# zpelgrims/pota

Measured on AMD Instinct MI355X. Metric: bidir redistribution Msamples/s at 4K, double-gauss 50mm, higher is better.
Workload: dtype f64

## Files before the change

### include/lentil_hip.h

```cpp
#ifndef LENTIL_HIP_H
#define LENTIL_HIP_H

#include <stddef.h>
#include <stdint.h>

#ifdef __cplusplus
extern "C" {
#endif

#define LENTIL_ABI_VERSION 1

#define LENTIL_OK 0
#define LENTIL_ERR_INVALID (-1)
#define LENTIL_ERR_HIP (-2)
#define LENTIL_ERR_UNSUPPORTED (-3)
#define LENTIL_ERR_NOMEM (-4)

#define LENTIL_THINLENS 0
#define LENTIL_POLYNOMIAL_OPTICS 1
#define LENTIL_UNIT_MM 0
#define LENTIL_UNIT_CM 1
#define LENTIL_UNIT_DM 2
#define LENTIL_UNIT_M 3
#define LENTIL_FILTER_GAUSSIAN 0
// ... 331 lines not shown
  uint64_t capacity;
  lentil_draw *out;
  double lambda;
  uint64_t *n_draws;
  uint64_t *attempts;
} lentil_draw_list;
int lentil_hip_list_draws(lentil_hip_ctx *ctx, const lentil_draw_list *list);
int lentil_hip_list_draws_path(lentil_hip_ctx *ctx, int *path);
int lentil_hip_draw_channels(const lentil_params *p, uint32_t *n_channels, double lambda[3], float rgb_weight[3][3]);

int lentil_hip_test_y0_intersection(lentil_hip_ctx *ctx, uint64_t n, const double *sensor_shift, double lambda,
                                    double *distance, double *sensor, double *out);
int lentil_hip_test_lt_sample_aperture(lentil_hip_ctx *ctx, uint64_t n, const double *scene,
                                       const double *ap, double lambda, double *sensor,
                                       double *out, double *transmittance);
int lentil_hip_test_trace_bw_po(lentil_hip_ctx *ctx, uint64_t n, const double *target,
                                const int32_t *px, const int32_t *py, const int32_t *attempt,
                                double *sensor_xy, int32_t *ok);
int lentil_hip_test_aperture_sample(lentil_hip_ctx *ctx, uint64_t n, const uint32_t *a,
                                    const uint32_t *b, double *xy);
int lentil_hip_test_xor128_jump(const uint32_t in[4], uint64_t k, uint32_t out[4]);
int lentil_hip_debug_scan_bands(const lentil_params *params, float out[8]);
int lentil_hip_debug_scan_lean_counts(uint32_t out[3]);
enum {
  LENTIL_SCAN_DMA2 = 1,
  LENTIL_SCAN_DMA = 2,
  LENTIL_SCAN_DMA_MULTI = 3,
  LENTIL_SCAN_UNIFORM = 4,
  LENTIL_SCAN_UNIFORM_MULTI = 5,
  LENTIL_SCAN_RUNS = 6,
// ... 9 lines not shown
```

### pota_amd/capi.py

```python
import ctypes as C
import os

import numpy as np

from . import _abi

_PKG = os.path.dirname(os.path.abspath(__file__))
LIB_PATH = os.environ.get("LENTIL_HIP_LIB") or os.path.join(_PKG, "liblentil_hip.so")

EXPORTS = [
    "lentil_hip_abi_version", "lentil_hip_create", "lentil_hip_destroy", "lentil_hip_last_error", "lentil_hip_last_redo_note",
    "lentil_hip_set_params", "lentil_hip_set_lens", "lentil_hip_set_bokeh", "lentil_hip_alloc_frame", "lentil_hip_set_camera_motion", "lentil_hip_set_camera_shutter",
    "lentil_hip_upload_visits", "lentil_hip_bind_visits", "lentil_hip_clear_frame",
    "lentil_hip_redistribute", "lentil_hip_resolve", "lentil_hip_sync", "lentil_hip_download_aov",
    "lentil_hip_download_accum", "lentil_hip_download_records", "lentil_hip_accum_buffer", "lentil_hip_stream",
    "lentil_hip_set_closest_exchange", "lentil_hip_zkey_buffer", "lentil_hip_closest_gather",
    "lentil_hip_touched_rows", "lentil_hip_merge_rows", "lentil_hip_resolve_rows",
    "lentil_hip_pack_rows", "lentil_hip_merge_packed_rows", "lentil_hip_compact_rows", "lentil_hip_merge_sparse",
    "lentil_hip_get_counters", "lentil_hip_last_timing", "lentil_hip_last_launches", "lentil_hip_set_draw_log",
    "lentil_hip_batch_model_stats", "lentil_hip_process_stats", "lentil_hip_process_stall_notes", "lentil_hip_set_async", "lentil_hip_pass_totals", "lentil_hip_set_occlusion_probe", "lentil_hip_probe_stats",
    "lentil_hip_set_occlusion_probe_device", "lentil_hip_probe_device_stats", "lentil_hip_test_sphere_occluder_device", "lentil_hip_debug_batch_estimate", "lentil_hip_box_probe",
    "lentil_hip_lens_jit_status", "lentil_hip_lens_jit_wait", "lentil_hip_debug_lens_jit_source", "lentil_hip_debug_lens_jit_compile",
    "lentil_hip_download_draw_log", "lentil_hip_test_lt_sample_aperture",
    "lentil_hip_test_trace_bw_po", "lentil_hip_test_aperture_sample", "lentil_hip_debug_scan_bands", "lentil_hip_debug_scan_lean_counts", "lentil_hip_debug_last_scan",
    "lentil_hip_lens_is_compiled", "lentil_hip_set_lens_mode",
    "lentil_hip_focus_search", "lentil_hip_test_y0_intersection", "lentil_hip_camera_rays", "lentil_hip_camera_rays_path",
    "lentil_hip_trace_points", "lentil_hip_trace_points_path",
    "lentil_hip_plan_visits", "lentil_hip_list_draws", "lentil_hip_list_draws_path", "lentil_hip_draw_channels",
    "lentil_hip_set_xor128_state", "lentil_hip_get_xor128_state", "lentil_hip_tl_chroma_stats", "lentil_hip_test_xor128_jump",
    "lentil_hip_host_alloc", "lentil_hip_host_free", "lentil_hip_visits_begin", "lentil_hip_visits_append",
    "lentil_hip_visits_wait", "lentil_hip_visits_end",
    "lentil_hip_comm_unique_id", "lentil_hip_comm_init", "lentil_hip_comm_destroy", "lentil_hip_allreduce",
    "lentil_hip_exchange_bands", "lentil_hip_exchange_stats", "lentil_hip_exchange_counts", "lentil_hip_degenerate_stats", "lentil_hip_streams_concurrent",
    "lentil_hip_alloc_crypto", "lentil_hip_upload_crypto", "lentil_hip_bind_crypto", "lentil_hip_download_crypto",
    "lentil_hip_download_crypto_table", "lentil_hip_visits_begin_crypto", "lentil_hip_visits_append_crypto",
]

SCAN_DMA2, SCAN_DMA, SCAN_DMA_MULTI, SCAN_UNIFORM, SCAN_UNIFORM_MULTI, SCAN_RUNS, SCAN_RAGGED = range(1, 8)
# ... 113 lines not shown
        "lentil_hip_lens_jit_wait": (i, [vp, C.c_double]),
        "lentil_hip_debug_lens_jit_compile": (i, [vp, i, C.c_char_p, C.c_uint64, C.POINTER(C.c_uint64), C.c_char_p, C.c_uint64,
                                                  C.POINTER(C.c_double), C.POINTER(C.c_uint64)]),
        "lentil_hip_debug_lens_jit_source": (i, [vp, C.c_char_p, C.c_uint64, C.POINTER(C.c_uint64)]),
        "lentil_hip_debug_batch_estimate": (i, [vp, C.c_uint64, vp, C.c_uint32, vp]),
        "lentil_hip_alloc_crypto": (i, [vp, u32, u32]),
        "lentil_hip_upload_crypto": (i, [vp, C.POINTER(_abi.CryptoVisits)]),
        "lentil_hip_bind_crypto": (i, [vp, C.POINTER(_abi.CryptoVisits)]),
        "lentil_hip_download_crypto": (i, [vp, u32, u32, vp, vp]),
        "lentil_hip_visits_begin_crypto": (i, [vp, u32]),
        "lentil_hip_visits_append_crypto": (i, [vp, C.POINTER(_abi.Visits), C.POINTER(_abi.CryptoVisits), C.POINTER(u64)]),
        "lentil_hip_download_crypto_table": (i, [vp, u32, C.POINTER(u32), vp, vp, vp]),
        "lentil_hip_set_draw_log": (i, [vp, u64]),
        "lentil_hip_download_draw_log": (i, [vp, vp, u64, C.POINTER(u64)]),
        "lentil_hip_test_lt_sample_aperture": (i, [vp, u64, vp, vp, C.c_double, vp, vp, vp]),
        "lentil_hip_test_trace_bw_po": (i, [vp, u64, vp, vp, vp, vp, vp, vp]),
        "lentil_hip_test_aperture_sample": (i, [vp, u64, vp, vp, vp]),
        "lentil_hip_lens_is_compiled": (i, [vp]),
        "lentil_hip_set_lens_mode": (i, [vp, i]),
        "lentil_hip_focus_search": (i, [vp, C.c_double, C.c_double, C.POINTER(C.c_double)]),
        "lentil_hip_camera_rays": (i, [vp, C.POINTER(_abi.CameraRayBatch)]),
        "lentil_hip_camera_rays_path": (i, [vp, C.POINTER(C.c_int)]),
        "lentil_hip_trace_points": (i, [vp, C.POINTER(_abi.PointBatch)]),
        "lentil_hip_trace_points_path": (i, [vp, C.POINTER(C.c_int)]),
        "lentil_hip_plan_visits": (i, [vp, u64, u64, vp, C.c_uint32, C.POINTER(u64)]),
        "lentil_hip_list_draws": (i, [vp, C.POINTER(_abi.DrawList)]),
        "lentil_hip_list_draws_path": (i, [vp, C.POINTER(C.c_int)]),
        "lentil_hip_draw_channels": (i, [C.POINTER(_abi.Params), C.POINTER(u32), C.POINTER(C.c_double), C.POINTER(C.c_float)]),
        "lentil_hip_set_xor128_state": (i, [vp, C.POINTER(C.c_uint32)]),
        "lentil_hip_get_xor128_state": (i, [vp, C.POINTER(C.c_uint32)]),
# ... 627 lines not shown
        self._chk(self.lib.lentil_hip_download_draw_log(self.h, None, 0, C.byref(n)))
        rec = np.empty((n.value, 3), np.uint32)
        if n.value:
            self._chk(self.lib.lentil_hip_download_draw_log(self.h, rec.ctypes.data, n.value, C.byref(n)))
        return rec

    def test_lt_sample_aperture(self, scene, ap, lam):
        scene = np.ascontiguousarray(scene, np.float64)
        ap = np.ascontiguousarray(ap, np.float64)
        n = scene.shape[0]
        sensor = np.empty((n, 5)); out = np.empty((n, 5)); T = np.empty((n,))
        self._chk(self.lib.lentil_hip_test_lt_sample_aperture(
            self.h, n, scene.ctypes.data, ap.ctypes.data, lam, sensor.ctypes.data, out.ctypes.data, T.ctypes.data))
        return sensor, out, T

    def test_trace_bw_po(self, target, px, py, attempt):
        target = np.ascontiguousarray(target, np.float64)
        px = np.ascontiguousarray(px, np.int32); py = np.ascontiguousarray(py, np.int32)
        attempt = np.ascontiguousarray(attempt, np.int32)
        n = target.shape[0]
        xy = np.empty((n, 2)); ok = np.empty((n,), np.int32)
        self._chk(self.lib.lentil_hip_test_trace_bw_po(
            self.h, n, target.ctypes.data, px.ctypes.data, py.ctypes.data, attempt.ctypes.data,
            xy.ctypes.data, ok.ctypes.data))
        return xy, ok

    def test_aperture_sample(self, a, b):
        a = np.ascontiguousarray(a, np.uint32); b = np.ascontiguousarray(b, np.uint32)
        xy = np.empty((a.shape[0], 2))
        self._chk(self.lib.lentil_hip_test_aperture_sample(self.h, a.shape[0], a.ctypes.data, b.ctypes.data,
# ... 3 lines not shown
```

### pota_amd/csrc/lentil_device.h

```cpp
#pragma once
#include <hip/hip_runtime.h>
#include <stdint.h>

#include "../../include/lentil_hip.h"

#define LD_DEV __device__ __forceinline__

namespace lentil {

constexpr float kAiPi = 3.14159265358979323846f;
constexpr float kAiPiOver2 = 1.57079632679489661923f;
constexpr float kAiEpsilon = 1.0e-4f;
constexpr float kAiInfinite = 1.0e30f;
constexpr double kPi = 3.14159265358979323846;

enum PolyId {
  P_OUT_X = 0, P_OUT_Y, P_OUT_DX, P_OUT_DY, P_OUT_T,
  P_AP_X, P_AP_Y, P_AP_DX, P_AP_DY,
  P_DAP_00, P_DAP_01, P_DAP_10, P_DAP_11,
  P_DOUT_00, P_DOUT_01, P_DOUT_10, P_DOUT_11,
  P_DAPPOS_00, P_DAPPOS_01, P_DAPPOS_10, P_DAPPOS_11,
  P_COUNT
};

// ... 160 lines not shown
  const double n2 = sqrt(fmax(0.0, R * R - ipx * ipx - ipy * ipy)) / fabs(R);
  const double t2 = sqrt(fmax(0.0, 1.0 - idx * idx - idy * idy));
  double ex0 = n2, ex1 = 0.0, ex2 = -n0;
  normalise3(ex0, ex1, ex2);
  const double ey0 = n1 * ex2 - n2 * ex1;
  const double ey1 = n2 * ex0 - n0 * ex2;
  const double ey2 = n0 * ex1 - n1 * ex0;
  dir[0] = idx * ex0 + idy * ey0 + t2 * n0;
  dir[1] = idx * ex1 + idy * ey1 + t2 * n1;
  dir[2] = idx * ex2 + idy * ey2 + t2 * n2;
  pos[0] = ipx;
  pos[1] = ipy;
  pos[2] = n2 * R + center;
}

LD_DEV void csToSphere(const double pos[3], double vx, double vy, double vz, double &odx, double &ody,
                       double center, double R) {
  const double n0 = pos[0] / R, n1 = pos[1] / R, n2 = fabs((pos[2] - center) / R);
  normalise3(vx, vy, vz);
  double ex0 = n2, ex1 = 0.0, ex2 = -n0;
  normalise3(ex0, ex1, ex2);
  const double ey0 = n1 * ex2 - n2 * ex1;
  const double ey1 = n2 * ex0 - n0 * ex2;
  const double ey2 = n0 * ex1 - n1 * ex0;
  odx = vx * ex0 + vy * ex1 + vz * ex2;
  ody = vx * ey0 + vy * ey1 + vz * ey2;
}

LD_DEV void cylinderToCs(double ipx, double ipy, double idx, double idy, double pos[3], double dir[3],
                         double center, double R, bool cyl_y) {
  double n0 = 0.0, n1 = 0.0, n2;
  if (cyl_y) { n0 = ipx / R; n2 = sqrt(fmax(0.0, R * R - ipx * ipx)) / fabs(R); }
  else { n1 = ipy / R; n2 = sqrt(fmax(0.0, R * R - ipy * ipy)) / fabs(R); }
  const double t2 = sqrt(fmax(0.0, 1.0 - idx * idx - idy * idy));
  double ex0 = n2, ex1 = 0.0, ex2 = -n0;
  normalise3(ex0, ex1, ex2);
  double ey0 = n1 * ex2 - n2 * ex1;
  double ey1 = n2 * ex0 - n0 * ex2;
  double ey2 = n0 * ex1 - n1 * ex0;
  normalise3(ey0, ey1, ey2);
  dir[0] = idx * ex0 + idy * ey0 + t2 * n0;
  dir[1] = idx * ex1 + idy * ey1 + t2 * n1;
  dir[2] = idx * ex2 + idy * ey2 + t2 * n2;
  pos[0] = ipx;
  pos[1] = ipy;
  pos[2] = n2 * R + center;
}

LD_DEV void csToCylinder(const double pos[3], double vx, double vy, double vz, double &odx, double &ody,
                         double center, double R, bool cyl_y) {
  double n0 = 0.0, n1 = 0.0;
  if (cyl_y) n0 = pos[0] / R; else n1 = pos[1] / R;
  const double n2 = fabs((pos[2] - center) / R);
  normalise3(vx, vy, vz);
  const double ex0 = n2, ex1 = 0.0, ex2 = -n0;
  double ey0 = n1 * ex2 - n2 * ex1;
  double ey1 = n2 * ex0 - n0 * ex2;
  double ey2 = n0 * ex1 - n1 * ex0;
  normalise3(ey0, ey1, ey2);
  odx = vx * ex0 + vy * ex1 + vz * ex2;
  ody = vx * ey0 + vy * ey1 + vz * ey2;
}

LD_DEV double ipow_u(double x, uint32_t e) {
  uint32_t odd = 0, n = 0;
  while (e > 2) { odd = (odd << 1) | (e & 1u); ++n; e >>= 1; }
  double p = (e == 2) ? x * x : x;
  for (uint32_t i = 0; i < n; ++i) {
    p = (odd & 1u) ? (x * p) * p : p * p;
    odd >>= 1;
  }
  return p;
}

struct LdsLens {
  const DevTerm *terms;
// ... 52 lines not shown
  int k, error;
};

LD_DEV void newton_init(NewtonState &s) {
  s.x = 0; s.y = 0; s.dx = 0; s.dy = 0;
  s.sqr_err = 1e30; s.sqr_ap_err = 1e30;
  s.out[0] = s.out[1] = s.out[2] = s.out[3] = 0.0;
  s.k = 0; s.error = 0;
}

LD_DEV bool newton_continue(const NewtonState &s) {
  const double eps = 1e-8;
  return s.k < 100 && (s.sqr_err > eps || s.sqr_ap_err > eps) && s.error == 0;
}

template <class Lens>
LD_DEV void newton_iter(const Lens &L, const double scene[3], double ap_x, double ap_y, NewtonState &s) {
  const DevLens &k = L.consts();
  const double R = k.outer_pupil_curvature_radius;
  const double prev_sqr_err = s.sqr_err, prev_sqr_ap_err = s.sqr_ap_err;
  const double begin[4] = {s.x, s.y, s.dx, s.dy};
  double pred_ap[2], Jap[4], Jout[4];
  L.eval_bw(begin, pred_ap, Jap, s.out, Jout);
  const double d0 = ap_x - pred_ap[0], d1 = ap_y - pred_ap[1];
  s.sqr_ap_err = d0 * d0 + d1 * d1;
  {
    const double invdet = 1.0 / (Jap[0] * Jap[3] - Jap[1] * Jap[2]);
    const double i00 = Jap[3] * invdet, i11 = Jap[0] * invdet;
    const double i01 = -Jap[1] * invdet, i10 = -Jap[2] * invdet;
    s.dx += i00 * d0; s.dy += i10 * d0;
    s.dx += i01 * d1; s.dy += i11 * d1;
  }
  double pos[3], dir[3];
  double on_dx, on_dy;
  if (k.outer_pupil_geometry == LENTIL_GEOM_SPHERICAL) {
    sphereToCs(s.out[0], s.out[1], s.out[2], s.out[3], pos, dir, -R, R);
    double vx = scene[0] - pos[0], vy = scene[1] - pos[1], vz = scene[2] - pos[2];
    normalise3(vx, vy, vz);
    csToSphere(pos, vx, vy, vz, on_dx, on_dy, -R, R);
  } else {
    const bool cy = k.outer_pupil_geometry == LENTIL_GEOM_CYL_Y;
    cylinderToCs(s.out[0], s.out[1], s.out[2], s.out[3], pos, dir, -R, R, cy);
    double vx = scene[0] - pos[0], vy = scene[1] - pos[1], vz = scene[2] - pos[2];
    normalise3(vx, vy, vz);
    csToCylinder(pos, vx, vy, vz, on_dx, on_dy, -R, R, cy);
  }
  const double e0 = on_dx - s.out[2], e1 = on_dy - s.out[3];
  s.sqr_err = e0 * e0 + e1 * e1;
  {
    const double invdet = 1.0 / (Jout[0] * Jout[3] - Jout[1] * Jout[2]);
    const double i00 = Jout[3] * invdet, i11 = Jout[0] * invdet;
    const double i01 = -Jout[1] * invdet, i10 = -Jout[2] * invdet;
    s.x += 0.72 * i00 * e0; s.y += 0.72 * i10 * e0;
    s.x += 0.72 * i01 * e1; s.y += 0.72 * i11 * e1;
  }
  int error = s.error;
  if (s.sqr_err > prev_sqr_err) error |= 1;
  if (s.sqr_ap_err > prev_sqr_ap_err) error |= 2;
  if (s.out[0] != s.out[0]) error |= 4;
  if (s.out[2] * s.out[2] + s.out[3] * s.out[3] > 1.0) error |= 8;
  if (s.k < 10) error = 0;
  s.error = error;
  s.k += 1;
}

template <class Lens>
LD_DEV double lens_evaluate(const Lens &L, const double in[4], double out[4]) {
  L.eval_out(in, out);
  return fmax(0.0, L.transmittance(in));
}

template <class Lens>
LD_DEV void lens_pt_sample_aperture(const Lens &L, double in[4], double ap_x, double ap_y, double dist,
                                    double &out_dx, double &out_dy) {
  double dx = in[2], dy = in[3];
  double pred_dx = 0.0, pred_dy = 0.0;
  double sqr_err = 3.4028234663852886e38;
  for (int k = 0; k < 5 && sqr_err > 1e-4; ++k) {
// ... 53 lines not shown
  } else {
    out4 = 0.0;
  }
  return fmax(0.0, out4);
}

template <class Lens>
LD_DEV double lt_sample_aperture(const Lens &L, const double scene[3], double ap_x, double ap_y,
                                 double sensor[4], double out[5], int *iters = nullptr) {
  NewtonState s;
  newton_init(s);
  while (newton_continue(s)) newton_iter(L, scene, ap_x, ap_y, s);
  const double T = newton_finish(L, s, out[4]);
  out[0] = s.out[0]; out[1] = s.out[1]; out[2] = s.out[2]; out[3] = s.out[3];
  if (iters) *iters = s.k;
  sensor[0] = s.x; sensor[1] = s.y; sensor[2] = s.dx; sensor[3] = s.dy;
  return T;
}

template <class Gen>
struct GenLens {
  const DevLens *k;
  LD_DEV void eval_bw(const double v[4], double pred_ap[2], double Jap[4], double out[4], double Jout[4]) const {
    Gen::eval_bw(v, k->lambda_pow, pred_ap, Jap, out, Jout);
  }
  LD_DEV double transmittance(const double v[4]) const { return Gen::transmittance(v, k->lambda_pow); }
  LD_DEV void eval_fw_newton(const double v[4], double pred_ap[2], double pred_dir[2], double Jap[4], double Jappos[4]) const {
    Gen::eval_fw_newton(v, k->lambda_pow, pred_ap, pred_dir, Jap, Jappos);
  }
  LD_DEV void eval_out(const double v[4], double out[4]) const { Gen::eval_out(v, k->lambda_pow, out); }
// ... 451 lines not shown
```

### pota_amd/csrc/lentil_hip.hip

```cpp
#include <hip/hip_runtime.h>
#include <hip/hip_ext.h>

#include <algorithm>
#include <atomic>
#include <chrono>
#include <cmath>
#include <cstdio>
#include <cstdlib>
#include <cstring>
#include <deque>
#include <mutex>
#include <new>
#include <string>
#include <vector>

#include "lentil_kernels.h"
#include "lentil_closest_replay.h"
#include "lentil_tl_chroma_mgpu.h"
#include "lentil_lens_jit.h"
#include "lentil_camera_rays.h"
#include "lentil_trace_points.h"
#include "lentil_list_draws.h"
#include "generated/embedded_sources.inc"

// ... 3467 lines not shown
                       ctx->extra_num, ctx->extra_const, d_out);
    hipError_t e = hipGetLastError();
    if (e == hipSuccess) e = hipStreamSynchronize(ctx->stream);
    if (e == hipSuccess) e = hipMemcpy(out, d_out, (size_t)n * 4 * sizeof(float), hipMemcpyDeviceToHost);
    if (e != hipSuccess) rc = fail(ctx, LENTIL_ERR_HIP, std::string("batch estimate: ") + hipGetErrorString(e));
  }
  for (void *p : tmp) (void)hipFree(p);
  return rc;
}

struct TmpFree {
  std::vector<void *> v;
  ~TmpFree() { for (void *p : v) (void)hipFree(p); }
};

LENTIL_API int lentil_hip_test_lt_sample_aperture(lentil_hip_ctx *ctx, uint64_t n, const double *scene,
                                                  const double *ap, double lambda, double *sensor,
                                                  double *out, double *transmittance) {
  CHECK_CTX(ctx);
  if (!ctx->have_lens) return fail(ctx, LENTIL_ERR_INVALID, "set_lens first");
  if (!n) return LENTIL_OK;
  HIP_TRY(ctx, hipSetDevice(ctx->device));
  TmpFree tf;
  TestArgs t{};
  t.P = ctx->P; t.lens = ctx->d_lens; t.terms = ctx->d_terms; t.bokeh = ctx->bokeh; t.n = n; t.lambda = lambda;
  double *d_scene, *d_ap, *o0, *o1, *o2;
  int rc;
  if ((rc = dev_copy_in(ctx, scene, n * 3, &d_scene, tf.v))) return rc;
  if ((rc = dev_copy_in(ctx, ap, n * 2, &d_ap, tf.v))) return rc;
  if ((rc = dev_alloc(ctx, n * 5, &o0, tf.v))) return rc;
  if ((rc = dev_alloc(ctx, n * 5, &o1, tf.v))) return rc;
  if ((rc = dev_alloc(ctx, n, &o2, tf.v))) return rc;
  t.in0 = d_scene; t.in1 = d_ap; t.o0 = o0; t.o1 = o1; t.o2 = o2;
  hipLaunchKernelGGL(test_kernel<0>, dim3((unsigned)((n + 255) / 256)), dim3(256), 0, ctx->stream, t);
  HIP_TRY(ctx, hipGetLastError());
  HIP_TRY(ctx, hipStreamSynchronize(ctx->stream));
  HIP_TRY(ctx, hipMemcpy(sensor, o0, n * 5 * 8, hipMemcpyDeviceToHost));
  HIP_TRY(ctx, hipMemcpy(out, o1, n * 5 * 8, hipMemcpyDeviceToHost));
  HIP_TRY(ctx, hipMemcpy(transmittance, o2, n * 8, hipMemcpyDeviceToHost));
  return LENTIL_OK;
}

static void focus_candidates(std::vector<double> &shift) {
  shift.clear();
  for (double i = -1.0; i <= 1.0; i += 0.0001) shift.push_back((i < 0 ? -1 : 1) * std::pow(i, 2.0) * (45.0 - 0.0) + 0.0);
}

static int run_focus(lentil_hip_ctx *ctx, const double *shift, uint32_t n, double focal_distance, double lambda,
                     double *miss, double *sensor, double *out, double *best) {
  TmpFree tf;
  FocusArgs f{};
  f.lens = ctx->d_lens; f.terms = ctx->d_terms; f.lambda = lambda; f.housing_radius = ctx->lens_housing_radius;
  f.focal_distance = focal_distance; f.n = n;
  double *d_shift, *d_miss, *d_sensor = nullptr, *d_out = nullptr, *d_best;
  int rc;
// ... 567 lines not shown
```

### pota_amd/csrc/lentil_kernels.h

```cpp
#pragma once
#include "lentil_device.h"
#include "lentil_batch_model.h"
#include "generated/lens_registry.h"

using namespace lentil;

struct DevCounters {
  unsigned long long work_count;
  unsigned long long sum_samples;
  unsigned long long redistributed;
  unsigned long long attempted;
  unsigned long long accepted;
  unsigned long long overflow;
  unsigned long long log_count;
  unsigned long long newton_iters;
  unsigned long long tries;
  unsigned long long lane_rounds;
  unsigned long long slow_solves;
  unsigned long long fallback;
  unsigned long long rounds_used;
  unsigned int n_tasks[2];
  unsigned int task_head[2];
  unsigned int n_active[2];
  unsigned int active_head[2];
// ... 1867 lines not shown
  double out4;
  const float transmittance = (float)newton_finish(L, s, out4);
  if (transmittance <= 0) return kCodeFail;
  const double ipx = s.x + s.dx * k.back_focal_length;
  const double ipy = s.y + s.dy * k.back_focal_length;
  if (ipx * ipx + ipy * ipy > k.inner_pupil_radius * k.inner_pupil_radius) return kCodeFail;
  const double sx = s.x + s.dx * -P.sensor_shift;
  const double sy = s.y + s.dy * -P.sensor_shift;
  uint32_t pix;
  return po_sensor_to_pixel(P, sx, sy, pix) ? pix : kCodeOut;
}

#ifndef LENTIL_SOLVE_ATTR
#define LENTIL_SOLVE_ATTR __attribute__((amdgpu_waves_per_eu(3)))
#endif
template <class LensT, bool kTables, bool kChroma = false, bool kStream = false>
__global__ __launch_bounds__(256) LENTIL_SOLVE_ATTR void solve_po_kernel(DrawArgs a) {
  LENTIL_TL_SPAN(a.round == 0 ? SPAN_SOLVE_R0 : (a.round == 1 ? SPAN_SOLVE_R1 : SPAN_SOLVE_R2));
  __shared__ DevTerm s_terms[kTables ? kMaxTerms : 1];
  __shared__ DevLens s_k;
  __shared__ DevLens s_kc[kChroma ? 3 : 1];
  __shared__ float s_cdfRow[kMaxBokehRows];
  __shared__ uint64_t s_hdr[4][4];
  __shared__ double s_ap[4][64][2];
  __shared__ double s_fin[4][6][64];
  __shared__ uint32_t s_fin_err[4][64], s_fin_res[4][64];
  if (kTables) {
    const uint32_t nt = a.lens->n_terms;
    for (uint32_t i = threadIdx.x; i < nt; i += blockDim.x) s_terms[i] = a.terms[i];
  }
  if (threadIdx.x == 0) s_k = *a.lens;
  if (kChroma && threadIdx.x < 3) {
    DevLens h = *a.lens;
    const double lam = a.lambda[threadIdx.x];
    h.lambda_pow[0] = 1.0; h.lambda_pow[1] = lam;
    for (uint32_t e = 2; e <= kMaxExp; ++e) h.lambda_pow[e] = ipow_u(lam, e);
    s_kc[threadIdx.x] = h;
  }
  const bool row_in_lds = a.P.bokeh_enable_image && a.bokeh.y <= kMaxBokehRows;
  if (row_in_lds)
    for (int i = threadIdx.x; i < a.bokeh.y; i += blockDim.x) s_cdfRow[i] = a.bokeh.cdfRow[i];
  __syncthreads();
  const float *cdfRow = row_in_lds ? s_cdfRow : a.bokeh.cdfRow;
  LensT L;
  if constexpr (kTables) { L.terms = s_terms; L.k = &s_k; } else { L.k = &s_k; }
  const DevLens &k = s_k;
  const lentil_params &P = a.P;

  if (blockIdx.x == 0 && threadIdx.x == 0 && !a.no_reset) reset_round(a.ctr, (uint32_t)a.parity ^ 1u);
  const uint32_t par = (uint32_t)a.parity;
  const Task *tasks = a.tasks[par];
  uint32_t *res = a.pool[par];
  uint32_t n_tasks = 0;
  if constexpr (!kStream) n_tasks = a.ctr->n_tasks[par] < a.task_cap ? a.ctr->n_tasks[par] : a.task_cap;
  const uint32_t lane = lane_id();
  const unsigned long long lt_mask = (1ull << lane) - 1ull;
  if (a.slow_live && a.slow && lane == 0) atomicAdd(&a.ctr->waves_started[par], 1u);
#ifdef LENTIL_PROBE_BUILD
  if (kStream && a.dispatch_probe && a.round == 1 && lane == 0) atomicAdd(&a.ctr->probe_res_xcc[0][xcc_id()], 1u);
#endif

  uint32_t cur_item = 0, cur_m = 0, cur_res = 0, cur_left = 0, cur_chan = 0;
  (void)cur_chan;
  bool no_more = false;
  constexpr uint32_t kNoTicket = 0xFFFFFFFFu;
  uint32_t ticket = kNoTicket, polls = 0;
  uint64_t ticket_t0 = 0;
  uint32_t idle_naps = 1u;
  (void)ticket; (void)polls; (void)ticket_t0; (void)idle_naps;
  bool busy = false;
  uint32_t res_idx = 0, cur_chan_lane = 0, my_item = 0;
  (void)cur_chan_lane;
  const uint32_t wv = threadIdx.x >> 6;
  uint32_t cur_pos = 0;
  uint32_t fin_n = 0;
  auto flush_finished = [&]() {
    if (fin_n == 0u) return;
    __builtin_amdgcn_fence(__ATOMIC_RELEASE, "wavefront", "local");
    __builtin_amdgcn_wave_barrier();
    __builtin_amdgcn_fence(__ATOMIC_ACQUIRE, "wavefront", "local");
    if (lane < fin_n) {
      NewtonState t;
      t.x = s_fin[wv][0][lane]; t.y = s_fin[wv][1][lane]; t.dx = s_fin[wv][2][lane]; t.dy = s_fin[wv][3][lane];
      t.out[0] = s_fin[wv][4][lane]; t.out[1] = s_fin[wv][5][lane]; t.out[2] = 0.0; t.out[3] = 0.0;
      t.sqr_err = 0.0; t.sqr_ap_err = 0.0; t.k = 0;
// ... 4 lines not shown
      res[s_fin_res[wv][lane]] = solve_result(P, Lf, t);
    }
    __builtin_amdgcn_fence(__ATOMIC_RELEASE, "wavefront", "local");
    __builtin_amdgcn_wave_barrier();
    fin_n = 0u;
  };
  auto start_task = [&]() {
    cur_pos = 0u;
    __builtin_amdgcn_fence(__ATOMIC_RELEASE, "wavefront", "local");
    __builtin_amdgcn_wave_barrier();
    __builtin_amdgcn_fence(__ATOMIC_ACQUIRE, "wavefront", "local");
    if (lane < cur_left) {
      double ax = 0.0, ay = 0.0;
      po_aperture_sample(P, a.bokeh, cdfRow, (uint32_t)s_hdr[wv][3], cur_m + lane, ax, ay);
      s_ap[wv][lane][0] = ax; s_ap[wv][lane][1] = ay;
    }
    __builtin_amdgcn_fence(__ATOMIC_RELEASE, "wavefront", "local");
    __builtin_amdgcn_wave_barrier();
    __builtin_amdgcn_fence(__ATOMIC_ACQUIRE, "wavefront", "local");
  };
  double target[3] = {0, 0, 1};
  double ap_x = 0.0, ap_y = 0.0;
  NewtonState s;
  newton_init(s);
  uint32_t st_iters = 0, st_tries = 0, st_rounds = 0;
  const bool parking = a.slow != nullptr && a.round >= a.slow_from_round && (kStream || a.ctr->sum_samples < a.slow_below);
  bool producers_gone = false;
  (void)producers_gone;

  while (true) {
// ... 68 lines not shown
          }
          if (cur_left == 0) continue;
        }
      }
      uint32_t take = n_idle - filled;
      if (take > cur_left) take = cur_left;
      if (!busy && my_rank >= filled && my_rank < filled + take) {
        const uint32_t j = my_rank - filled;
        res_idx = cur_res + j;
        const uint64_t *hs = s_hdr[wv];
        target[0] = __longlong_as_double((long long)hs[0]);
        target[1] = __longlong_as_double((long long)hs[1]);
        target[2] = __longlong_as_double((long long)hs[2]);
        ap_x = s_ap[wv][cur_pos + j][0];
        ap_y = s_ap[wv][cur_pos + j][1];
        newton_init(s);
        ++st_tries;
        busy = true;
        my_item = cur_item;
        if constexpr (kChroma) { L.k = &s_kc[cur_chan]; cur_chan_lane = cur_chan; }
      }
      cur_pos += take; cur_res += take; cur_left -= take; filled += take;
    }
    if (inflight + filled == 0u) {
      flush_finished();
      if (!kStream || no_more) break;
      for (uint32_t i = 0; i < idle_naps; ++i) __builtin_amdgcn_s_sleep(127);
      if (idle_naps < 8u) idle_naps <<= 1;
      continue;
    }
    idle_naps = 1u;

    if (busy) { newton_iter(L, target, ap_x, ap_y, s); ++st_iters; }
    ++st_rounds;
#ifdef LENTIL_TIMELINE
    { const uint32_t nb_ = (uint32_t)__builtin_popcountll(__ballot(busy)); if (lane == 0) tl_add(!kStream || a.round ? TL_ITERS_LATER : (a.instance ? TL_ITERS_B : TL_ITERS_A), nb_); }
#endif

    {
      const bool fin = busy && !newton_continue(s);
      const unsigned long long fmask = __ballot(fin);
      if (fmask) {
        const uint32_t nfin = (uint32_t)__builtin_popcountll(fmask);
        if (fin_n + nfin > 64u) flush_finished();
        if (fin) {
          const uint32_t q = fin_n + (uint32_t)__builtin_popcountll(fmask & lt_mask);
          s_fin[wv][0][q] = s.x; s_fin[wv][1][q] = s.y; s_fin[wv][2][q] = s.dx; s_fin[wv][3][q] = s.dy;
          s_fin[wv][4][q] = s.out[0]; s_fin[wv][5][q] = s.out[1];
// ... 2095 lines not shown
  const uint32_t *u0, *u1;
  double lambda;
  double *o0, *o1, *o2;
  int32_t *oi;
};

template <int WHAT>
__global__ __launch_bounds__(256) void test_kernel(TestArgs t) {
  __shared__ DevTerm s_terms[kMaxTerms];
  __shared__ DevLens s_k;
  if (t.lens) {
    const uint32_t nt = t.lens->n_terms;
    for (uint32_t i = threadIdx.x; i < nt; i += blockDim.x) s_terms[i] = t.terms[i];
    if (threadIdx.x == 0) {
      s_k = *t.lens;
      if (WHAT == 0) {
        s_k.lambda_pow[0] = 1.0; s_k.lambda_pow[1] = t.lambda;
        for (uint32_t e = 2; e <= kMaxExp; ++e) s_k.lambda_pow[e] = ipow_u(t.lambda, e);
      }
    }
  }
  __syncthreads();
  const LdsLens L{s_terms, &s_k};
  const uint64_t i = (uint64_t)blockIdx.x * blockDim.x + threadIdx.x;
  const uint64_t ii = i < t.n ? i : t.n - 1;
  if (WHAT == 0) {
    double sensor[4], out[5] = {0, 0, 0, 0, t.lambda};
    const double scene[3] = {t.in0[ii * 3], t.in0[ii * 3 + 1], t.in0[ii * 3 + 2]};
    int iters = 0;
    const double T = lt_sample_aperture(L, scene, t.in1[ii * 2], t.in1[ii * 2 + 1], sensor, out, &iters);
    if (i < t.n) {
      for (int c = 0; c < 4; ++c) t.o0[i * 5 + c] = sensor[c];
      t.o0[i * 5 + 4] = t.lambda;
      for (int c = 0; c < 5; ++c) t.o1[i * 5 + c] = out[c];
      t.o2[i] = T;
      if (t.oi) t.oi[i] = iters;
    }
  } else if (WHAT == 1) {
    const double target[3] = {t.in0[ii * 3], t.in0[ii * 3 + 1], t.in0[ii * 3 + 2]};
    double sx = 0, sy = 0;
    const bool ok = trace_ray_bw_po(t.P, L, t.bokeh, t.bokeh.cdfRow, target, t.i0[ii], t.i1[ii], t.i2[ii], sx, sy);
    if (i < t.n) { t.o0[i * 2] = sx; t.o0[i * 2 + 1] = sy; t.oi[i] = ok ? 1 : 0; }
  } else {
    double ax, ay;
    po_aperture_sample(t.P, t.bokeh, t.bokeh.cdfRow, t.u0[ii], t.u1[ii], ax, ay);
// ... 5 lines not shown
```

### pota_amd/csrc/lentil_scan.h

```cpp
#pragma once

static ScanBands scan_bands(const lentil_params &P) {
  ScanBands B;
  for (int i = 0; i < 2; ++i) { B.in_lo[i] = 1.0f; B.in_hi[i] = -1.0f; B.out_lo[i] = 1.0f; B.out_hi[i] = -1.0f; }
  B.out_lo[0] = -INFINITY; B.out_hi[0] = INFINITY;
  float fd = (float)P.focus_distance, A = (float)P.aperture_radius;
  if (P.cameraType == LENTIL_POLYNOMIAL_OPTICS) fd = (float)((double)fd / 10.0);
  else A = (float)((double)A * 10.0);
  const float f = P.focal_length;
  const float ifd = (-f * -fd) / (-f + -fd);
  const double a = std::fabs((double)A), c0 = 1.0 + (double)ifd / (double)f, c1 = (double)ifd;
  if (!(a > 0.0) || !std::isfinite(a) || !std::isfinite(c0) || !std::isfinite(c1) || c1 == 0.0 || !(f > 0.0f)) return B;
  const double eps = 1e-3 + 1e-5 * a;
  if (!(eps < 0.25)) return B;
  auto up = [](double v) { float r = (float)v; if ((double)r < v) r = std::nextafter(r, INFINITY); return r; };
  auto down = [](double v) { float r = (float)v; if ((double)r > v) r = std::nextafter(r, -INFINITY); return r; };
  auto pieces = [&](double t, bool inner, float lo[2], float hi[2]) {
    double ua = (c0 - t / a) / c1, ub = (c0 + t / a) / c1;
    if (ua > ub) std::swap(ua, ub);
    lo[0] = lo[1] = 1.0f; hi[0] = hi[1] = -1.0f;
    const double big = inner ? 1e30 : (double)INFINITY;
    if (ua > 0.0 || ub < 0.0) {
      const double zl = 1.0 / ub, zh = 1.0 / ua;
      lo[0] = inner ? up(std::max(zl, -big)) : down(zl);
// ... 44 lines not shown
static uint32_t dma_multi_blocks_per_cu(const lentil_hip_ctx *ctx) {
  static const int forced = getenv("LENTIL_DMA_MULTI_BLOCKS") ? atoi(getenv("LENTIL_DMA_MULTI_BLOCKS")) : 0;
  if (forced >= 1 && forced <= 4) return (uint32_t)forced;
  return 2u * dma_multi_lds(ctx) + 2u * 10u * 1024u <= 160u * 1024u ? 2u : 1u;
}

static bool dma_multi_applies(const lentil_hip_ctx *ctx) {
  static const bool allowed = !(getenv("LENTIL_SCAN_DMA_MULTI") && getenv("LENTIL_SCAN_DMA_MULTI")[0] == '0');
  const uint32_t M = ctx->V.visits_per_pixel;
  return allowed && ctx->scan_dma && M > 0 && M <= 64 && ctx->V.n_extra > 0 && !ctx->V.inv_density && !ctx->F.zkey && !ctx->F.zkey_dbg &&
         ctx->F.closest_mask == 0 && ctx->V.cam.n < 2 && ctx->V.n % M == 0 && dma_multi_lds(ctx) <= 160u * 1024u;
}

static size_t solve_block_lds(lentil_hip_ctx *ctx) {
  const bool straight = ctx->use_generated && (lentil_hip_lens_is_compiled(ctx) || jit_function(ctx, false, true) != nullptr);
  return straight ? 29184u : 53760u;
}
static bool fits_cu_beside_solves(size_t scan_lds, unsigned n_solve, size_t solve_lds, size_t slack) {
  return scan_lds + slack + (size_t)n_solve * solve_lds <= 160u * 1024u;
}

static int plan_scan(lentil_hip_ctx *ctx, ScanPlan &pl) {
  ScanArgs &sa = pl.sa;
  sa.P = ctx->P;
  sa.lens_length = ctx->have_lens ? ctx->hlens.length : 0.0;
  sa.V = ctx->V;
  sa.F = ctx->F;
  const uint32_t M = ctx->V.visits_per_pixel;
  pl.M = M;
  bool direct = false;
  if (M) {
// ... 135 lines not shown
```

Measured before the change: 42220.

## Hoist first Newton iteration's scene-independent work into per-block origin precompute

The first Newton iteration always starts from a zero state, so the polynomial evaluation, Jacobian inverses and pupil frame at that origin are the same for every sample. The solve kernel now computes them once per block (per channel for chroma), keeps them in LDS, computes the scene-dependent part once per wave item, and seeds each lane's state from them instead of running a full first iteration. This removes one full polynomial evaluation per solve, at the cost of extra LDS, a block-wide sync at kernel start, and a bit more per-item work. Test entry points are added to check the split path against the original.

```diff
diff --git a/include/lentil_hip.h b/include/lentil_hip.h
--- a/include/lentil_hip.h
+++ b/include/lentil_hip.h
@@ -369,6 +369,11 @@
 int lentil_hip_test_lt_sample_aperture(lentil_hip_ctx *ctx, uint64_t n, const double *scene,
                                        const double *ap, double lambda, double *sensor,
                                        double *out, double *transmittance);
+int lentil_hip_test_lt_sample_aperture_split(lentil_hip_ctx *ctx, uint64_t n, const double *scene,
+                                             const double *ap, double lambda, double *sensor,
+                                             double *out, double *transmittance);
+int lentil_hip_test_lt_sample_aperture_iters(lentil_hip_ctx *ctx, uint64_t n, const double *scene,
+                                             const double *ap, double lambda, int32_t split, int32_t *iters);
 int lentil_hip_test_trace_bw_po(lentil_hip_ctx *ctx, uint64_t n, const double *target,
                                 const int32_t *px, const int32_t *py, const int32_t *attempt,
                                 double *sensor_xy, int32_t *ok);
diff --git a/pota_amd/capi.py b/pota_amd/capi.py
--- a/pota_amd/capi.py
+++ b/pota_amd/capi.py
@@ -22,6 +22,7 @@
     "lentil_hip_set_occlusion_probe_device", "lentil_hip_probe_device_stats", "lentil_hip_test_sphere_occluder_device", "lentil_hip_debug_batch_estimate", "lentil_hip_box_probe",
     "lentil_hip_lens_jit_status", "lentil_hip_lens_jit_wait", "lentil_hip_debug_lens_jit_source", "lentil_hip_debug_lens_jit_compile",
     "lentil_hip_download_draw_log", "lentil_hip_test_lt_sample_aperture",
+    "lentil_hip_test_lt_sample_aperture_split", "lentil_hip_test_lt_sample_aperture_iters",
     "lentil_hip_test_trace_bw_po", "lentil_hip_test_aperture_sample", "lentil_hip_debug_scan_bands", "lentil_hip_debug_scan_lean_counts", "lentil_hip_debug_last_scan",
     "lentil_hip_lens_is_compiled", "lentil_hip_set_lens_mode",
     "lentil_hip_focus_search", "lentil_hip_test_y0_intersection", "lentil_hip_camera_rays", "lentil_hip_camera_rays_path",
@@ -165,6 +166,8 @@
         "lentil_hip_set_draw_log": (i, [vp, u64]),
         "lentil_hip_download_draw_log": (i, [vp, vp, u64, C.POINTER(u64)]),
         "lentil_hip_test_lt_sample_aperture": (i, [vp, u64, vp, vp, C.c_double, vp, vp, vp]),
+        "lentil_hip_test_lt_sample_aperture_split": (i, [vp, u64, vp, vp, C.c_double, vp, vp, vp]),
+        "lentil_hip_test_lt_sample_aperture_iters": (i, [vp, u64, vp, vp, C.c_double, C.c_int32, vp]),
         "lentil_hip_test_trace_bw_po": (i, [vp, u64, vp, vp, vp, vp, vp, vp]),
         "lentil_hip_test_aperture_sample": (i, [vp, u64, vp, vp, vp]),
         "lentil_hip_lens_is_compiled": (i, [vp]),
@@ -822,6 +825,23 @@
             self.h, n, scene.ctypes.data, ap.ctypes.data, lam, sensor.ctypes.data, out.ctypes.data, T.ctypes.data))
         return sensor, out, T
 
+    def test_lt_sample_aperture_split(self, scene, ap, lam):
+        scene = np.ascontiguousarray(scene, np.float64)
+        ap = np.ascontiguousarray(ap, np.float64)
+        n = scene.shape[0]
+        sensor = np.empty((n, 5)); out = np.empty((n, 5)); T = np.empty((n,))
+        self._chk(self.lib.lentil_hip_test_lt_sample_aperture_split(
+            self.h, n, scene.ctypes.data, ap.ctypes.data, lam, sensor.ctypes.data, out.ctypes.data, T.ctypes.data))
+        return sensor, out, T
+
+    def test_lt_sample_aperture_iters(self, scene, ap, lam, split):
+        scene = np.ascontiguousarray(scene, np.float64)
+        ap = np.ascontiguousarray(ap, np.float64)
+        it = np.empty((scene.shape[0],), np.int32)
+        self._chk(self.lib.lentil_hip_test_lt_sample_aperture_iters(
+            self.h, scene.shape[0], scene.ctypes.data, ap.ctypes.data, lam, 1 if split else 0, it.ctypes.data))
+        return it
+
     def test_trace_bw_po(self, target, px, py, attempt):
         target = np.ascontiguousarray(target, np.float64)
         px = np.ascontiguousarray(px, np.int32); py = np.ascontiguousarray(py, np.int32)
diff --git a/pota_amd/csrc/lentil_device.h b/pota_amd/csrc/lentil_device.h
--- a/pota_amd/csrc/lentil_device.h
+++ b/pota_amd/csrc/lentil_device.h
@@ -198,17 +198,31 @@
   pos[2] = n2 * R + center;
 }
 
+struct PupilFrame {
+  double ex[3], ey[3];
+};
+
+LD_DEV void pupilProject(const PupilFrame &f, double vx, double vy, double vz, double &odx, double &ody) {
+  normalise3(vx, vy, vz);
+  odx = vx * f.ex[0] + vy * f.ex[1] + vz * f.ex[2];
+  ody = vx * f.ey[0] + vy * f.ey[1] + vz * f.ey[2];
+}
+
+LD_DEV void sphereFrame(const double pos[3], double center, double R, PupilFrame &f) {
+  const double n0 = pos[0] / R, n1 = pos[1] / R, n2 = fabs((pos[2] - center) / R);
+  double ex0 = n2, ex1 = 0.0, ex2 = -n0;
+  normalise3(ex0, ex1, ex2);
+  f.ex[0] = ex0; f.ex[1] = ex1; f.ex[2] = ex2;
+  f.ey[0] = n1 * ex2 - n2 * ex1;
+  f.ey[1] = n2 * ex0 - n0 * ex2;
+  f.ey[2] = n0 * ex1 - n1 * ex0;
+}
+
 LD_DEV void csToSphere(const double pos[3], double vx, double vy, double vz, double &odx, double &ody,
                        double center, double R) {
-  const double n0 = pos[0] / R, n1 = pos[1] / R, n2 = fabs((pos[2] - center) / R);
-  normalise3(vx, vy, vz);
-  double ex0 = n2, ex1 = 0.0, ex2 = -n0;
-  normalise3(ex0, ex1, ex2);
-  const double ey0 = n1 * ex2 - n2 * ex1;
-  const double ey1 = n2 * ex0 - n0 * ex2;
-  const double ey2 = n0 * ex1 - n1 * ex0;
-  odx = vx * ex0 + vy * ex1 + vz * ex2;
-  ody = vx * ey0 + vy * ey1 + vz * ey2;
+  PupilFrame f;
+  sphereFrame(pos, center, R, f);
+  pupilProject(f, vx, vy, vz, odx, ody);
 }
 
 LD_DEV void cylinderToCs(double ipx, double ipy, double idx, double idy, double pos[3], double dir[3],
@@ -231,19 +245,24 @@
   pos[2] = n2 * R + center;
 }
 
-LD_DEV void csToCylinder(const double pos[3], double vx, double vy, double vz, double &odx, double &ody,
-                         double center, double R, bool cyl_y) {
+LD_DEV void cylinderFrame(const double pos[3], double center, double R, bool cyl_y, PupilFrame &f) {
   double n0 = 0.0, n1 = 0.0;
   if (cyl_y) n0 = pos[0] / R; else n1 = pos[1] / R;
   const double n2 = fabs((pos[2] - center) / R);
-  normalise3(vx, vy, vz);
   const double ex0 = n2, ex1 = 0.0, ex2 = -n0;
   double ey0 = n1 * ex2 - n2 * ex1;
   double ey1 = n2 * ex0 - n0 * ex2;
   double ey2 = n0 * ex1 - n1 * ex0;
   normalise3(ey0, ey1, ey2);
-  odx = vx * ex0 + vy * ex1 + vz * ex2;
-  ody = vx * ey0 + vy * ey1 + vz * ey2;
+  f.ex[0] = ex0; f.ex[1] = ex1; f.ex[2] = ex2;
+  f.ey[0] = ey0; f.ey[1] = ey1; f.ey[2] = ey2;
+}
+
+LD_DEV void csToCylinder(const double pos[3], double vx, double vy, double vz, double &odx, double &ody,
+                         double center, double R, bool cyl_y) {
+  PupilFrame f;
+  cylinderFrame(pos, center, R, cyl_y, f);
+  pupilProject(f, vx, vy, vz, odx, ody);
 }
 
 LD_DEV double ipow_u(double x, uint32_t e) {
@@ -326,10 +345,34 @@
   return s.k < 100 && (s.sqr_err > eps || s.sqr_ap_err > eps) && s.error == 0;
 }
 
+LD_DEV void newton_inverse(const double J[4], double i[4]) {
+  const double invdet = 1.0 / (J[0] * J[3] - J[1] * J[2]);
+  const double i00 = J[3] * invdet, i11 = J[0] * invdet;
+  const double i01 = -J[1] * invdet, i10 = -J[2] * invdet;
+  i[0] = i00; i[1] = i01; i[2] = i10; i[3] = i11;
+}
+
+LD_DEV void newton_pupil_point(const DevLens &k, const double out[4], double pos[3], PupilFrame &f) {
+  const double R = k.outer_pupil_curvature_radius;
+  double dir[3];
+  if (k.outer_pupil_geometry == LENTIL_GEOM_SPHERICAL) {
+    sphereToCs(out[0], out[1], out[2], out[3], pos, dir, -R, R);
+    sphereFrame(pos, -R, R, f);
+  } else {
+    const bool cy = k.outer_pupil_geometry == LENTIL_GEOM_CYL_Y;
+    cylinderToCs(out[0], out[1], out[2], out[3], pos, dir, -R, R, cy);
+    cylinderFrame(pos, -R, R, cy, f);
+  }
+}
+LD_DEV void newton_pupil_dir(const double pos[3], const PupilFrame &f, const double scene[3], double &on_dx, double &on_dy) {
+  double vx = scene[0] - pos[0], vy = scene[1] - pos[1], vz = scene[2] - pos[2];
+  normalise3(vx, vy, vz);
+  pupilProject(f, vx, vy, vz, on_dx, on_dy);
+}
+
 template <class Lens>
 LD_DEV void newton_iter(const Lens &L, const double scene[3], double ap_x, double ap_y, NewtonState &s) {
   const DevLens &k = L.consts();
-  const double R = k.outer_pupil_curvature_radius;
   const double prev_sqr_err = s.sqr_err, prev_sqr_ap_err = s.sqr_ap_err;
   const double begin[4] = {s.x, s.y, s.dx, s.dy};
   double pred_ap[2], Jap[4], Jout[4];
@@ -337,34 +380,22 @@
   const double d0 = ap_x - pred_ap[0], d1 = ap_y - pred_ap[1];
   s.sqr_ap_err = d0 * d0 + d1 * d1;
   {
-    const double invdet = 1.0 / (Jap[0] * Jap[3] - Jap[1] * Jap[2]);
-    const double i00 = Jap[3] * invdet, i11 = Jap[0] * invdet;
-    const double i01 = -Jap[1] * invdet, i10 = -Jap[2] * invdet;
-    s.dx += i00 * d0; s.dy += i10 * d0;
-    s.dx += i01 * d1; s.dy += i11 * d1;
-  }
-  double pos[3], dir[3];
-  double on_dx, on_dy;
-  if (k.outer_pupil_geometry == LENTIL_GEOM_SPHERICAL) {
-    sphereToCs(s.out[0], s.out[1], s.out[2], s.out[3], pos, dir, -R, R);
-    double vx = scene[0] - pos[0], vy = scene[1] - pos[1], vz = scene[2] - pos[2];
-    normalise3(vx, vy, vz);
-    csToSphere(pos, vx, vy, vz, on_dx, on_dy, -R, R);
-  } else {
-    const bool cy = k.outer_pupil_geometry == LENTIL_GEOM_CYL_Y;
-    cylinderToCs(s.out[0], s.out[1], s.out[2], s.out[3], pos, dir, -R, R, cy);
-    double vx = scene[0] - pos[0], vy = scene[1] - pos[1], vz = scene[2] - pos[2];
-    normalise3(vx, vy, vz);
-    csToCylinder(pos, vx, vy, vz, on_dx, on_dy, -R, R, cy);
-  }
+    double i[4];
+    newton_inverse(Jap, i);
+    s.dx += i[0] * d0; s.dy += i[2] * d0;
+    s.dx += i[1] * d1; s.dy += i[3] * d1;
+  }
+  double pos[3], on_dx, on_dy;
+  PupilFrame f;
+  newton_pupil_point(k, s.out, pos, f);
+  newton_pupil_dir(pos, f, scene, on_dx, on_dy);
   const double e0 = on_dx - s.out[2], e1 = on_dy - s.out[3];
   s.sqr_err = e0 * e0 + e1 * e1;
   {
-    const double invdet = 1.0 / (Jout[0] * Jout[3] - Jout[1] * Jout[2]);
-    const double i00 = Jout[3] * invdet, i11 = Jout[0] * invdet;
-    const double i01 = -Jout[1] * invdet, i10 = -Jout[2] * invdet;
-    s.x += 0.72 * i00 * e0; s.y += 0.72 * i10 * e0;
-    s.x += 0.72 * i01 * e1; s.y += 0.72 * i11 * e1;
+    double i[4];
+    newton_inverse(Jout, i);
+    s.x += 0.72 * i[0] * e0; s.y += 0.72 * i[2] * e0;
+    s.x += 0.72 * i[1] * e1; s.y += 0.72 * i[3] * e1;
   }
   int error = s.error;
   if (s.sqr_err > prev_sqr_err) error |= 1;
@@ -374,6 +405,56 @@
   if (s.k < 10) error = 0;
   s.error = error;
   s.k += 1;
+}
+
+struct NewtonOrigin {
+  double pred_ap[2];
+  double iap[4];
+  double out[4];
+  double iout72[4];
+  double pos[3];
+  PupilFrame frame;
+};
+struct NewtonItem {
+  double x, y, sqr_err;
+};
+
+template <class Lens>
+LD_DEV void newton_origin(const Lens &L, NewtonOrigin &o) {
+  double begin[4] = {0.0, 0.0, 0.0, 0.0};
+#pragma unroll
+  for (int c = 0; c < 4; ++c) asm volatile("" : "+v"(begin[c]));
+  double Jap[4], Jout[4], i[4];
+  L.eval_bw(begin, o.pred_ap, Jap, o.out, Jout);
+  newton_inverse(Jap, o.iap);
+  newton_inverse(Jout, i);
+#pragma unroll
+  for (int c = 0; c < 4; ++c) o.iout72[c] = 0.72 * i[c];
+  newton_pupil_point(L.consts(), o.out, o.pos, o.frame);
+}
+
+LD_DEV NewtonItem newton_first_item(const NewtonOrigin &o, const double scene[3]) {
+  double on_dx, on_dy;
+  newton_pupil_dir(o.pos, o.frame, scene, on_dx, on_dy);
+  const double e0 = on_dx - o.out[2], e1 = on_dy - o.out[3];
+  NewtonItem it;
+  it.sqr_err = e0 * e0 + e1 * e1;
+  it.x = 0.0; it.y = 0.0;
+  it.x += o.iout72[0] * e0; it.y += o.iout72[2] * e0;
+  it.x += o.iout72[1] * e1; it.y += o.iout72[3] * e1;
+  return it;
+}
+
+LD_DEV void newton_first_unit(const NewtonOrigin &o, const NewtonItem &it, double ap_x, double ap_y, NewtonState &s) {
+  const double d0 = ap_x - o.pred_ap[0], d1 = ap_y - o.pred_ap[1];
+  s.sqr_ap_err = d0 * d0 + d1 * d1;
+  s.dx = 0.0; s.dy = 0.0;
+  s.dx += o.iap[0] * d0; s.dy += o.iap[2] * d0;
+  s.dx += o.iap[1] * d1; s.dy += o.iap[3] * d1;
+  s.x = it.x; s.y = it.y;
+  s.sqr_err = it.sqr_err;
+  s.out[0] = o.out[0]; s.out[1] = o.out[1]; s.out[2] = o.out[2]; s.out[3] = o.out[3];
+  s.k = 1; s.error = 0;
 }
 
 template <class Lens>
@@ -457,6 +538,22 @@
   const double T = newton_finish(L, s, out[4]);
   out[0] = s.out[0]; out[1] = s.out[1]; out[2] = s.out[2]; out[3] = s.out[3];
   if (iters) *iters = s.k;
+  sensor[0] = s.x; sensor[1] = s.y; sensor[2] = s.dx; sensor[3] = s.dy;
+  return T;
+}
+
+template <class Lens>
+LD_DEV double lt_sample_aperture_split(const Lens &L, const double scene[3], double ap_x, double ap_y,
+                                       double sensor[4], double out[5], int *iters = nullptr) {
+  NewtonOrigin o;
+  newton_origin(L, o);
+  const NewtonItem it = newton_first_item(o, scene);
+  NewtonState s;
+  newton_first_unit(o, it, ap_x, ap_y, s);
+  while (newton_continue(s)) newton_iter(L, scene, ap_x, ap_y, s);
+  const double T = newton_finish(L, s, out[4]);
+  out[0] = s.out[0]; out[1] = s.out[1]; out[2] = s.out[2]; out[3] = s.out[3];
+  if (iters) *iters = s.k - 1;
   sensor[0] = s.x; sensor[1] = s.y; sensor[2] = s.dx; sensor[3] = s.dy;
   return T;
 }
diff --git a/pota_amd/csrc/lentil_hip.hip b/pota_amd/csrc/lentil_hip.hip
--- a/pota_amd/csrc/lentil_hip.hip
+++ b/pota_amd/csrc/lentil_hip.hip
@@ -3505,10 +3505,10 @@
   ~TmpFree() { for (void *p : v) (void)hipFree(p); }
 };
 
-LENTIL_API int lentil_hip_test_lt_sample_aperture(lentil_hip_ctx *ctx, uint64_t n, const double *scene,
-                                                  const double *ap, double lambda, double *sensor,
-                                                  double *out, double *transmittance) {
-  CHECK_CTX(ctx);
+static int run_lt_sample_aperture(lentil_hip_ctx *ctx, uint64_t n, const double *scene, const double *ap, double lambda, bool split,
+                                  double *sensor, double *out, double *transmittance, int32_t *iters) {
+  CHECK_CTX(ctx);
+  if (!scene || !ap) return fail(ctx, LENTIL_ERR_INVALID, "null argument");
   if (!ctx->have_lens) return fail(ctx, LENTIL_ERR_INVALID, "set_lens first");
   if (!n) return LENTIL_OK;
   HIP_TRY(ctx, hipSetDevice(ctx->device));
@@ -3522,14 +3522,36 @@
   if ((rc = dev_alloc(ctx, n * 5, &o0, tf.v))) return rc;
   if ((rc = dev_alloc(ctx, n * 5, &o1, tf.v))) return rc;
   if ((rc = dev_alloc(ctx, n, &o2, tf.v))) return rc;
-  t.in0 = d_scene; t.in1 = d_ap; t.o0 = o0; t.o1 = o1; t.o2 = o2;
-  hipLaunchKernelGGL(test_kernel<0>, dim3((unsigned)((n + 255) / 256)), dim3(256), 0, ctx->stream, t);
+  int32_t *oi = nullptr;
+  if (iters && (rc = dev_alloc(ctx, n, &oi, tf.v))) return rc;
+  t.in0 = d_scene; t.in1 = d_ap; t.o0 = o0; t.o1 = o1; t.o2 = o2; t.oi = oi;
+  if (split) hipLaunchKernelGGL(test_kernel<3>, dim3((unsigned)((n + 255) / 256)), dim3(256), 0, ctx->stream, t);
+  else hipLaunchKernelGGL(test_kernel<0>, dim3((unsigned)((n + 255) / 256)), dim3(256), 0, ctx->stream, t);
   HIP_TRY(ctx, hipGetLastError());
   HIP_TRY(ctx, hipStreamSynchronize(ctx->stream));
-  HIP_TRY(ctx, hipMemcpy(sensor, o0, n * 5 * 8, hipMemcpyDeviceToHost));
-  HIP_TRY(ctx, hipMemcpy(out, o1, n * 5 * 8, hipMemcpyDeviceToHost));
-  HIP_TRY(ctx, hipMemcpy(transmittance, o2, n * 8, hipMemcpyDeviceToHost));
-  return LENTIL_OK;
+  if (sensor) HIP_TRY(ctx, hipMemcpy(sensor, o0, n * 5 * 8, hipMemcpyDeviceToHost));
+  if (out) HIP_TRY(ctx, hipMemcpy(out, o1, n * 5 * 8, hipMemcpyDeviceToHost));
+  if (transmittance) HIP_TRY(ctx, hipMemcpy(transmittance, o2, n * 8, hipMemcpyDeviceToHost));
+  if (iters) HIP_TRY(ctx, hipMemcpy(iters, oi, n * 4, hipMemcpyDeviceToHost));
+  return LENTIL_OK;
+}
+
+LENTIL_API int lentil_hip_test_lt_sample_aperture(lentil_hip_ctx *ctx, uint64_t n, const double *scene,
+                                                  const double *ap, double lambda, double *sensor,
+                                                  double *out, double *transmittance) {
+  return run_lt_sample_aperture(ctx, n, scene, ap, lambda, false, sensor, out, transmittance, nullptr);
+}
+
+LENTIL_API int lentil_hip_test_lt_sample_aperture_split(lentil_hip_ctx *ctx, uint64_t n, const double *scene,
+                                                        const double *ap, double lambda, double *sensor,
+                                                        double *out, double *transmittance) {
+  return run_lt_sample_aperture(ctx, n, scene, ap, lambda, true, sensor, out, transmittance, nullptr);
+}
+
+LENTIL_API int lentil_hip_test_lt_sample_aperture_iters(lentil_hip_ctx *ctx, uint64_t n, const double *scene,
+                                                        const double *ap, double lambda, int32_t split, int32_t *iters) {
+  if (ctx && !iters) return fail(ctx, LENTIL_ERR_INVALID, "null argument");
+  return run_lt_sample_aperture(ctx, n, scene, ap, lambda, split != 0, nullptr, nullptr, nullptr, iters);
 }
 
 static void focus_candidates(std::vector<double> &shift) {
diff --git a/pota_amd/csrc/lentil_kernels.h b/pota_amd/csrc/lentil_kernels.h
--- a/pota_amd/csrc/lentil_kernels.h
+++ b/pota_amd/csrc/lentil_kernels.h
@@ -1905,17 +1905,40 @@
 #ifndef LENTIL_SOLVE_ATTR
 #define LENTIL_SOLVE_ATTR __attribute__((amdgpu_waves_per_eu(3)))
 #endif
+template <bool kTables, bool kChroma>
+struct SolveShared {
+  DevTerm terms[kTables ? kMaxTerms : 1];
+  DevLens k;
+  DevLens kc[kChroma ? 3 : 1];
+  float cdfRow[kMaxBokehRows];
+  uint64_t hdr[4][4];
+  double ap[4][64][2];
+  double fin[4][6][64];
+  uint32_t fin_err[4][64], fin_res[4][64];
+  NewtonOrigin origin[kChroma ? 3 : 1];
+  NewtonItem item[4];
+};
+constexpr size_t kSolveLdsStraight = 29184, kSolveLdsTables = 53760;
+static_assert(sizeof(SolveShared<false, false>) <= kSolveLdsStraight && sizeof(SolveShared<false, true>) <= kSolveLdsStraight,
+              "a resident solve block outgrew the LDS the streamed pass plans with (solve_block_lds)");
+static_assert(sizeof(SolveShared<true, false>) <= kSolveLdsTables && sizeof(SolveShared<true, true>) <= kSolveLdsTables,
+              "a resident solve block outgrew the LDS the streamed pass plans with (solve_block_lds)");
+
 template <class LensT, bool kTables, bool kChroma = false, bool kStream = false>
 __global__ __launch_bounds__(256) LENTIL_SOLVE_ATTR void solve_po_kernel(DrawArgs a) {
   LENTIL_TL_SPAN(a.round == 0 ? SPAN_SOLVE_R0 : (a.round == 1 ? SPAN_SOLVE_R1 : SPAN_SOLVE_R2));
-  __shared__ DevTerm s_terms[kTables ? kMaxTerms : 1];
-  __shared__ DevLens s_k;
-  __shared__ DevLens s_kc[kChroma ? 3 : 1];
-  __shared__ float s_cdfRow[kMaxBokehRows];
-  __shared__ uint64_t s_hdr[4][4];
-  __shared__ double s_ap[4][64][2];
-  __shared__ double s_fin[4][6][64];
-  __shared__ uint32_t s_fin_err[4][64], s_fin_res[4][64];
+  __shared__ SolveShared<kTables, kChroma> sh;
+  auto &s_terms = sh.terms;
+  DevLens &s_k = sh.k;
+  auto &s_kc = sh.kc;
+  auto &s_cdfRow = sh.cdfRow;
+  auto &s_hdr = sh.hdr;
+  auto &s_ap = sh.ap;
+  auto &s_fin = sh.fin;
+  auto &s_fin_err = sh.fin_err;
+  auto &s_fin_res = sh.fin_res;
+  auto &s_origin = sh.origin;
+  auto &s_item = sh.item;
   if (kTables) {
     const uint32_t nt = a.lens->n_terms;
     for (uint32_t i = threadIdx.x; i < nt; i += blockDim.x) s_terms[i] = a.terms[i];
@@ -1937,6 +1960,15 @@
   if constexpr (kTables) { L.terms = s_terms; L.k = &s_k; } else { L.k = &s_k; }
   const DevLens &k = s_k;
   const lentil_params &P = a.P;
+  if ((threadIdx.x >> 6) < (kChroma ? 3u : 1u)) {
+    const uint32_t c = threadIdx.x >> 6;
+    LensT Lo = L;
+    if constexpr (kChroma) Lo.k = &s_kc[c];
+    NewtonOrigin o;
+    newton_origin(Lo, o);
+    if ((threadIdx.x & 63u) == 0u) s_origin[c] = o;
+  }
+  __syncthreads();
 
   if (blockIdx.x == 0 && threadIdx.x == 0 && !a.no_reset) reset_round(a.ctr, (uint32_t)a.parity ^ 1u);
   const uint32_t par = (uint32_t)a.parity;
@@ -1960,6 +1992,7 @@
   uint32_t idle_naps = 1u;
   (void)ticket; (void)polls; (void)ticket_t0; (void)idle_naps;
   bool busy = false;
+  bool first_ends = false;
   uint32_t res_idx = 0, cur_chan_lane = 0, my_item = 0;
   (void)cur_chan_lane;
   const uint32_t wv = threadIdx.x >> 6;
@@ -1994,6 +2027,13 @@
       double ax = 0.0, ay = 0.0;
       po_aperture_sample(P, a.bokeh, cdfRow, (uint32_t)s_hdr[wv][3], cur_m + lane, ax, ay);
       s_ap[wv][lane][0] = ax; s_ap[wv][lane][1] = ay;
+    }
+    {
+      const uint64_t *hs = s_hdr[wv];
+      const double scene[3] = {__longlong_as_double((long long)hs[0]), __longlong_as_double((long long)hs[1]),
+                               __longlong_as_double((long long)hs[2])};
+      const NewtonItem it = newton_first_item(s_origin[kChroma ? cur_chan : 0u], scene);
+      if (lane == 0u) s_item[wv] = it;
     }
     __builtin_amdgcn_fence(__ATOMIC_RELEASE, "wavefront", "local");
     __builtin_amdgcn_wave_barrier();
@@ -2092,7 +2132,8 @@
         target[2] = __longlong_as_double((long long)hs[2]);
         ap_x = s_ap[wv][cur_pos + j][0];
         ap_y = s_ap[wv][cur_pos + j][1];
-        newton_init(s);
+        newton_first_unit(s_origin[kChroma ? cur_chan : 0u], s_item[wv], ap_x, ap_y, s);
+        first_ends = !newton_continue(s);
         ++st_tries;
         busy = true;
         my_item = cur_item;
@@ -2109,7 +2150,7 @@
     }
     idle_naps = 1u;
 
-    if (busy) { newton_iter(L, target, ap_x, ap_y, s); ++st_iters; }
+    if (busy && !first_ends) { newton_iter(L, target, ap_x, ap_y, s); ++st_iters; }
     ++st_rounds;
 #ifdef LENTIL_TIMELINE
     { const uint32_t nb_ = (uint32_t)__builtin_popcountll(__ballot(busy)); if (lane == 0) tl_add(!kStream || a.round ? TL_ITERS_LATER : (a.instance ? TL_ITERS_B : TL_ITERS_A), nb_); }
@@ -4235,7 +4276,7 @@
     for (uint32_t i = threadIdx.x; i < nt; i += blockDim.x) s_terms[i] = t.terms[i];
     if (threadIdx.x == 0) {
       s_k = *t.lens;
-      if (WHAT == 0) {
+      if (WHAT == 0 || WHAT == 3) {
         s_k.lambda_pow[0] = 1.0; s_k.lambda_pow[1] = t.lambda;
         for (uint32_t e = 2; e <= kMaxExp; ++e) s_k.lambda_pow[e] = ipow_u(t.lambda, e);
       }
@@ -4245,11 +4286,12 @@
   const LdsLens L{s_terms, &s_k};
   const uint64_t i = (uint64_t)blockIdx.x * blockDim.x + threadIdx.x;
   const uint64_t ii = i < t.n ? i : t.n - 1;
-  if (WHAT == 0) {
+  if (WHAT == 0 || WHAT == 3) {
     double sensor[4], out[5] = {0, 0, 0, 0, t.lambda};
     const double scene[3] = {t.in0[ii * 3], t.in0[ii * 3 + 1], t.in0[ii * 3 + 2]};
     int iters = 0;
-    const double T = lt_sample_aperture(L, scene, t.in1[ii * 2], t.in1[ii * 2 + 1], sensor, out, &iters);
+    const double T = WHAT == 3 ? lt_sample_aperture_split(L, scene, t.in1[ii * 2], t.in1[ii * 2 + 1], sensor, out, &iters)
+                               : lt_sample_aperture(L, scene, t.in1[ii * 2], t.in1[ii * 2 + 1], sensor, out, &iters);
     if (i < t.n) {
       for (int c = 0; c < 4; ++c) t.o0[i * 5 + c] = sensor[c];
       t.o0[i * 5 + 4] = t.lambda;
diff --git a/pota_amd/csrc/lentil_scan.h b/pota_amd/csrc/lentil_scan.h
--- a/pota_amd/csrc/lentil_scan.h
+++ b/pota_amd/csrc/lentil_scan.h
@@ -82,7 +82,7 @@
 
 static size_t solve_block_lds(lentil_hip_ctx *ctx) {
   const bool straight = ctx->use_generated && (lentil_hip_lens_is_compiled(ctx) || jit_function(ctx, false, true) != nullptr);
-  return straight ? 29184u : 53760u;
+  return straight ? kSolveLdsStraight : kSolveLdsTables;
 }
 static bool fits_cu_beside_solves(size_t scan_lds, unsigned n_solve, size_t solve_lds, size_t slack) {
   return scan_lds + slack + (size_t)n_solve * solve_lds <= 160u * 1024u;
```

New measurement: 43500 (median of 6 runs). 3.0% higher.
